# zhiyuns/REHRSeg

Measured on AMD Instinct MI355X. Metric: 3D patches/sec (fwd+bwd, 128^3 fp32), higher is better.
Workload: dtype f32; 1 GPU; FLAVR UNet_3D_3D(1,'unet_18',128,4) fwd+bwd+Adam, 1x1x128^3 patch per GPU, random-init weights; patches_per_gpu=1, global_batch=1, parallelism=dp1 (patch-parallel, flat-bucket RCCL all-reduce), wgrad_stream=True

## Files before the change

include/rehrseg_hip.h:

```cpp
#ifndef REHRSEG_HIP_H
#define REHRSEG_HIP_H

#include <stdint.h>

#ifdef __cplusplus
extern "C" {
#endif

#define REHR_OK 0
#define REHR_EINVAL -1
#define REHR_ENOSUP -2
#define REHR_EHIP -3

#define REHR_ACT_NONE 0
#define REHR_ACT_RELU 1
#define REHR_ACT_LRELU 2

typedef struct {
  int32_t count, off0, offs, k0, ks;
} rehr_axis_taps;

typedef struct {
  const float* x1;
  const float* x2;
// ... 39 lines not shown
#define REHR_GG_ROUTE_FLAT8 1
#define REHR_GG_ROUTE_W32P 2
#define REHR_GG_ROUTE_BIG8 3
#define REHR_GG_ROUTE_SMALL 4
#define REHR_GG_ROUTE_FLAT22 5
#define REHR_GG_ROUTE_REGION22 6
int rehr_gather_gemm_wino_route(const rehr_gather_gemm_desc* d);
#define REHR_GG_DIRECT_NONE 0
#define REHR_GG_DIRECT_GENERIC 1
#define REHR_GG_DIRECT_HALO 2
#define REHR_GG_DIRECT_TCONV_KS 3
int rehr_gather_gemm_direct_route(const rehr_gather_gemm_desc* descs, int32_t count, int32_t bf16, int32_t* routes);
int rehr_gather_gemm_f32(const rehr_gather_gemm_desc* d, void* stream);
int rehr_gather_gemm_multi_f32(const rehr_gather_gemm_desc* descs, int32_t count,
                               void* stream);
int rehr_gather_gemm_bf16(const rehr_gather_gemm_desc* d, void* stream);
int rehr_gather_gemm_multi_bf16(const rehr_gather_gemm_desc* descs, int32_t count, void* stream);
int rehr_pack_weights_bf16(const float* in, void* out, int32_t A, int32_t Apad, int32_t B, int32_t T,
                           int32_t transpose_ab, void* stream);

int rehr_sum_slabs_bias_act_f32(const float* slabs, int32_t S, int64_t slab_stride,
                                const float* bias, float* y, int64_t rows, int32_t C,
                                int32_t act, float slope, void* stream);

int rehr_sum_slabs_stats_f32(const float* slabs, int32_t S, int64_t slab_stride, const float* bias,
                             float* y, int32_t N, int64_t SV, int32_t C, int32_t act, float slope,
                             double* stats, void* stream);

int rehr_sum_slabs_bias_act_bf16(const float* slabs, int32_t S, int64_t slab_stride, const float* bias, void* y,
                                 int64_t rows, int32_t C, int32_t act, float slope, void* stream);
// ... 326 lines not shown
```

rehrseg_amd/csrc/gather_gemm.hip:

```cpp
#include "common.h"
#include "halo_shared.h"
#include "wino_shared.h"

namespace {

constexpr int BK = 32;
constexpr int LDS_LD = 36;
constexpr int NTHREADS = 256;

template <int BM, int BN, int WGM, int WGN, int LDSBUF>
__device__ __forceinline__ void gather_gemm_body(const GGParams& p, const int nblocks, const int logical_in = -1) {
  constexpr int WTM = BM / WGM, WTN = BN / WGN;
  constexpr int FM = WTM / 32, FN = WTN / 32;
  constexpr int AROWS = BM / 32, BROWS = BN / 32;
  static_assert(WGM * WGN == 4, "4 waves");
  const rehr_gather_gemm_desc& d = p.d;

  extern __shared__ __attribute__((aligned(16))) float smem[];
  float* As = smem;
  float* Bs = smem + LDSBUF * BM * LDS_LD;
  int* row_out = (int*)(Bs + LDSBUF * BN * LDS_LD);

  const int tid = threadIdx.x;
  const int lane = tid & 63, wave = tid >> 6;
// ... 290 lines not shown
  if (npad % 64 == 0) return launch_gg<128, 64, 2, 2, 1>(pm, count, st);
  return launch_gg<128, 32, 4, 1, 1>(pm, count, st);
}

}

WinoRoute wino_route(const rehr_gather_gemm_desc& d, WinoPlan& plan) {
  if (!(d.debug_flags & REHR_DBG_GG_NO_FLAT8) && wino_flat8_plan(d, plan)) return WINO_FLAT8;
  if (const WinoRoute r = wino_region_plan(d, plan)) return r;
  if (wino22_flat_plan(d, plan, 1)) return WINO_FLAT22;
  if (wino22_region_plan(d, plan)) return WINO_REGION22;
  plan.bytes = 0;
  return WINO_NONE;
}

static int wino_run(WinoRoute r, const rehr_gather_gemm_desc* ds, int count, const WinoPlan& plan, hipStream_t st) {
  for (int i = 0; i < count; ++i) {
    const int rc = r >= WINO_FLAT22 ? wino22_weights_launch(ds[i], plan, st) : wino_weights_launch(r, ds[i], plan, st);
    if (rc != REHR_OK) return rc;
  }
  if (ds[0].flags & REHR_GG_WS_ONLY) return REHR_OK;
  switch (r) {
    case WINO_FLAT8: return wino_flat8_launch(ds[0], plan, st);
    case WINO_W32P: case WINO_BIG8: case WINO_SMALL: return wino_region_launch(r, ds, count, plan, st);
    default: return wino22_launch(r, ds, count, plan, st);
  }
}

extern "C" int rehr_gather_gemm_multi_f32(const rehr_gather_gemm_desc* descs, int32_t count, void* stream) {
  DirectRoute route[MAX_PHASES];
  const int rrc = direct_route(descs, count, 4, route);
  if (rrc != REHR_OK) return rrc;
  hipStream_t st = (hipStream_t)stream;
  const bool ws_only = (descs[0].flags & REHR_GG_WS_ONLY) != 0;
  for (int i = 1; i < count; ++i)
    if ((descs[i].flags ^ descs[0].flags) & (REHR_GG_WS_ONLY | REHR_GG_WS_READY)) return REHR_EINVAL;
  if (route[0].kind == DIRECT_TCONV_KS && !ws_only) return tconv_ks_launch(descs, count, false, st);
  WinoPlan plan{};
  if (count > 1 && descs[0].wino_ws != nullptr) {
    const int taps = descs[0].td.count;
    if ((taps > 3 || taps == 1) && wino_split_plan(descs, count, plan)) return wino_run(WINO_BIG8, descs, count, plan, st);
    if (taps <= 3 && wino22_flat_multi_plan(descs, count, plan)) return wino_run(WINO_FLAT22, descs, count, plan, st);
  }
  GGMulti pm;
  pm.interleave = 0;
  pm.count = 0;
  pm.no_interleave = (descs[0].debug_flags & REHR_DBG_GG_INTERLEAVE) ? 0 : 1;
  int n = 0;
  for (int i = 0; i < count; ++i) {
    if (descs[i].wino_ws != nullptr && !(count > 1 && descs[i].td.count > 3)) {
      const WinoRoute r = wino_route(descs[i], plan);
      if (r != WINO_NONE && wino_ws_ok(descs[i], plan.bytes)) {
        const int wrc = wino_run(r, &descs[i], 1, plan, st);
        if (wrc != REHR_OK) return wrc;
        continue;
      }
    }
    if (ws_only) continue;
    if (route[i].kind == DIRECT_HALO) {
      const int hrc = halo_f32_launch(route[i].halo, st);
      if (hrc != REHR_OK) return hrc;
    } else if (route[i].kind == DIRECT_GENERIC) {
      pm.ph[n++] = route[i].gg;
    } else {
      return REHR_ENOSUP;
    }
  }
  if (n == 0) return REHR_OK;
  return launch_generic(pm, n, st);
}

extern "C" int64_t rehr_gather_gemm_wino_bytes(const rehr_gather_gemm_desc* dp) {
  WinoPlan plan{};
  if (dp == nullptr || validate(*dp) != REHR_OK || wino_route(*dp, plan) == WINO_NONE) return 0;
  return plan.bytes;
}

extern "C" int rehr_gather_gemm_wino_route(const rehr_gather_gemm_desc* dp) {
  WinoPlan plan{};
  if (dp == nullptr || validate(*dp) != REHR_OK) return REHR_GG_ROUTE_NONE;
  const WinoRoute r = wino_route(*dp, plan);
  return r == WINO_NONE ? REHR_GG_ROUTE_NONE : (int)r | (plan.variant << 8);
}

extern "C" int rehr_gather_gemm_direct_route(const rehr_gather_gemm_desc* descs, int32_t count, int32_t bf16,
                                             int32_t* routes) {
// ... 13 lines not shown
```

rehrseg_amd/csrc/wino22_conv.hip:

```cpp
#include "common.h"
#include "wino_shared.h"
#include <cstdlib>

namespace {

constexpr int LD = WINO_LDX;
constexpr int PW = 17;
constexpr int RP = PW * LD + 12;
constexpr int BUF = PW * RP;
constexpr int PVOX = PW * PW;
constexpr int NT_ = 768;
constexpr int NX = (PVOX * 8 + NT_ - 1) / NT_;
constexpr int MAXPH = WINO_MAXPH;

struct W22Params {
  rehr_gather_gemm_desc d;
  int nb_h, nb_w, kchunks, nphase;
  Phase phase[MAXPH];
  const float* up;
  uint32_t up_bytes;
};

__global__ void w22_weights_kernel(const rehr_gather_gemm_desc d, float* __restrict__ up, int kchunks) {
  AxisPlan ah, aw;
// ... 8 lines not shown
  for (int64_t i = (int64_t)blockIdx.x * blockDim.x + threadIdx.x; i < total; i += (int64_t)gridDim.x * blockDim.x) {
    const int pj = (int)(i / per);
    const int p = pj / d.td.count, jd = pj - p * d.td.count;
    const int p_h = p / aw.nph, p_w = p - p_h * aw.nph;
    const int64_t rem = i - (int64_t)pj * per;
    const int n = (int)(rem / cpad), ci = (int)(rem - (int64_t)n * cpad);
    float g[2][2];
#pragma unroll
    for (int a = 0; a < 2; ++a)
#pragma unroll
      for (int b = 0; b < 2; ++b) {
        const int wt = ((d.td.k0 + d.td.ks * jd) * d.KH + ah.kidx[p_h][a]) * d.KW + aw.kidx[p_w][b];
        g[a][b] = ci < d.Cin ? d.wp[(int64_t)wt * per_src + (int64_t)n * d.Cin + ci] : 0.f;
      }
    float u[9];
    u[0] = g[0][0];              u[1] = g[0][0] + g[0][1];                     u[2] = g[0][1];
    u[3] = g[0][0] + g[1][0];    u[4] = g[0][0] + g[0][1] + g[1][0] + g[1][1]; u[5] = g[0][1] + g[1][1];
    u[6] = g[1][0];              u[7] = g[1][0] + g[1][1];                     u[8] = g[1][1];
    const int nt = n >> 5, col = n & 31, chunk = ci >> 5, kk = (ci >> 3) & 3, half = (ci >> 2) & 1, e = ci & 3;
#pragma unroll
    for (int x = 0; x < 9; ++x) {
      const int64_t o = (((((int64_t)pj * 9 + x) * NT + nt) * kchunks + chunk) * 4 + kk) * 256 + (half * 32 + col) * 4 + e;
      up[o] = u[x];
    }
  }
}

__global__ __launch_bounds__(NT_) void wino22_conv_kernel(const W22Params p) {
  const rehr_gather_gemm_desc& d = p.d;
  extern __shared__ __attribute__((aligned(16))) float smem[];
  float* Xs = smem;

  const int tid = threadIdx.x, lane = tid & 63;
// ... 629 lines not shown
```

rehrseg_amd/csrc/wino_conv.hip:

```cpp
#include "common.h"
#include "wino_shared.h"
#include <cstdlib>

namespace {

constexpr int TH = 4, TW = 8;
constexpr int PH = 2 * TH + 2, PW = 2 * TW + 2;
constexpr int PVOX = PH * PW;
constexpr int LDX = 36;
constexpr int NX = (PVOX * 8 + 255) / 256;

struct WinoParams {
  rehr_gather_gemm_desc d;
  int nb_h, nb_w;
  int band_major;
  int kchunks;
  int dh0, dw0;
  const float* up;
  uint32_t up_bytes;
  int nsplit;
  rehr_axis_taps s_td[8];
  const float* s_up[8];
  uint32_t s_up_bytes[8];
  float* s_y[8];
};

__global__ void wino_weights_kernel(const rehr_gather_gemm_desc d, float* __restrict__ up) {
  const float G[4][3] = {{1.f, 0.f, 0.f}, {.5f, .5f, .5f}, {.5f, -.5f, .5f}, {0.f, 0.f, 1.f}};
  const int64_t per = (int64_t)d.Npad * d.Cin;
  const int64_t total = (int64_t)d.td.count * per;
  for (int64_t i = (int64_t)blockIdx.x * blockDim.x + threadIdx.x; i < total; i += (int64_t)gridDim.x * blockDim.x) {
    const int jd = (int)(i / per);
    const int64_t nc = i - (int64_t)jd * per;
    float g[3][3];
#pragma unroll
    for (int jh = 0; jh < 3; ++jh)
#pragma unroll
      for (int jw = 0; jw < 3; ++jw) {
        const int a = d.bh + d.th.off0 + d.th.offs * jh + 1;
        const int b = d.bw + d.tw.off0 + d.tw.offs * jw + 1;
        const int wt = ((d.td.k0 + d.td.ks * jd) * d.KH + (d.th.k0 + d.th.ks * jh)) * d.KW + (d.tw.k0 + d.tw.ks * jw);
        const float v = d.wp[(int64_t)wt * per + nc];
#pragma unroll
        for (int aa = 0; aa < 3; ++aa)
#pragma unroll
          for (int bb = 0; bb < 3; ++bb)
            if (aa == a && bb == b) g[aa][bb] = v;
      }
    float t[4][3];
#pragma unroll
    for (int r = 0; r < 4; ++r)
#pragma unroll
      for (int b = 0; b < 3; ++b) t[r][b] = G[r][0] * g[0][b] + G[r][1] * g[1][b] + G[r][2] * g[2][b];
#pragma unroll
    for (int r = 0; r < 4; ++r)
#pragma unroll
      for (int c = 0; c < 4; ++c)
        up[((int64_t)jd * 16 + r * 4 + c) * per + nc] = t[r][0] * G[c][0] + t[r][1] * G[c][1] + t[r][2] * G[c][2];
  }
}

__global__ __launch_bounds__(256, 2) void wino_conv_kernel(const WinoParams p) {
  const rehr_gather_gemm_desc& d = p.d;
  extern __shared__ __attribute__((aligned(16))) float smem[];
  float* Xs = smem;

  const int tid = threadIdx.x, lane = tid & 63;
  const int r = __builtin_amdgcn_readfirstlane(tid >> 6);
  const int half = lane >> 5, col = lane & 31;
  const int n_img = blockIdx.z;
  const int n0 = blockIdx.y * 32;
  int b = xcd_remap(blockIdx.x, gridDim.x);
  const int bw_ = b % p.nb_w; b /= p.nb_w;
// ... 169 lines not shown
    if (r == 0 && half == 0 && colok) {
      const float a1 = red[col] + red[64 + col] + red[128 + col] + red[192 + col];
      const float a2 = red[32 + col] + red[96 + col] + red[160 + col] + red[224 + col];
      double* st = d.stats + ((int64_t)n_img * d.Cout + col_n) * 2;
      atomicAdd(st, (double)a1);
      if (d.stats_mode == 2) atomicAdd(st + 1, (double)a2);
    }
  }
}

constexpr int PW2 = 18, PVOX2 = 18 * 18;
constexpr int RP2 = PW2 * LDX + 8;
constexpr int BUF2 = PW2 * RP2;

__global__ void wino_weights_frag_kernel(const rehr_gather_gemm_desc d, float* __restrict__ up, int kchunks) {
  const float G[4][3] = {{1.f, 0.f, 0.f}, {.5f, .5f, .5f}, {.5f, -.5f, .5f}, {0.f, 0.f, 1.f}};
  const int cpad = kchunks * 32;
  const int64_t per = (int64_t)d.Npad * cpad;
  const int64_t per_src = (int64_t)d.Npad * d.Cin;
  const int64_t total = (int64_t)d.td.count * per;
  const int NT = d.Npad / 32;
  for (int64_t i = (int64_t)blockIdx.x * blockDim.x + threadIdx.x; i < total; i += (int64_t)gridDim.x * blockDim.x) {
    const int jd = (int)(i / per);
    const int64_t rem = i - (int64_t)jd * per;
    const int n = (int)(rem / cpad), ci = (int)(rem - (int64_t)n * cpad);
    float g[3][3];
#pragma unroll
    for (int jh = 0; jh < 3; ++jh)
#pragma unroll
      for (int jw = 0; jw < 3; ++jw) {
        const int a = d.bh + d.th.off0 + d.th.offs * jh + 1;
        const int b = d.bw + d.tw.off0 + d.tw.offs * jw + 1;
        const int wt = ((d.td.k0 + d.td.ks * jd) * d.KH + (d.th.k0 + d.th.ks * jh)) * d.KW + (d.tw.k0 + d.tw.ks * jw);
        const float v = ci < d.Cin ? d.wp[(int64_t)wt * per_src + (int64_t)n * d.Cin + ci] : 0.f;
#pragma unroll
        for (int aa = 0; aa < 3; ++aa)
#pragma unroll
          for (int bb = 0; bb < 3; ++bb)
            if (aa == a && bb == b) g[aa][bb] = v;
      }
    float t[4][3];
#pragma unroll
    for (int r = 0; r < 4; ++r)
#pragma unroll
      for (int b = 0; b < 3; ++b) t[r][b] = G[r][0] * g[0][b] + G[r][1] * g[1][b] + G[r][2] * g[2][b];
    const int nt = n >> 5, col = n & 31, chunk = ci >> 5, kk = (ci >> 3) & 3, half = (ci >> 2) & 1, e = ci & 3;
#pragma unroll
    for (int r = 0; r < 4; ++r)
#pragma unroll
      for (int c = 0; c < 4; ++c) {
        const int64_t o = (((((int64_t)jd * 16 + r * 4 + c) * NT + nt) * kchunks + chunk) * 4 + kk) * 256 +
                          (half * 32 + col) * 4 + e;
        up[o] = t[r][0] * G[c][0] + t[r][1] * G[c][1] + t[r][2] * G[c][2];
      }
  }
}

constexpr int NX8 = (PVOX2 * 8 + 511) / 512;

__global__ __launch_bounds__(512) void wino_conv_big8_kernel(const WinoParams p) {
  const rehr_gather_gemm_desc& d = p.d;
  extern __shared__ __attribute__((aligned(16))) float smem[];
  float* Xs = smem;
  constexpr int BUF = BUF2;

  const int tid = threadIdx.x, lane = tid & 63;
  const int wv = __builtin_amdgcn_readfirstlane(tid >> 6);
  const int r = wv & 3, fm = wv >> 2;
  const int half = lane >> 5, col = lane & 31;
// ... 694 lines not shown
```

rehrseg_amd/csrc/wino_shared.h:

```cpp
#pragma once
#include "common.h"
#include "gg_shared.h"
#include "wino22_shared.h"

enum WinoRoute {
  WINO_NONE = REHR_GG_ROUTE_NONE,
  WINO_FLAT8 = REHR_GG_ROUTE_FLAT8,
  WINO_W32P = REHR_GG_ROUTE_W32P,
  WINO_BIG8 = REHR_GG_ROUTE_BIG8,
  WINO_SMALL = REHR_GG_ROUTE_SMALL,
  WINO_FLAT22 = REHR_GG_ROUTE_FLAT22,
  WINO_REGION22 = REHR_GG_ROUTE_REGION22,
};

constexpr int WINO_LDX = 36;
constexpr int WINO_MAXPH = 4;

struct Phase {
  int sh, sw;
  int ph, pw;
  int dh0, dw0;
};

struct FlatGeom {
// ... 112 lines not shown
    return a.count == b.count && a.off0 == b.off0 && a.offs == b.offs && a.k0 == b.k0 && a.ks == b.ks;
  };
  if ((groups & SAME_HW_TAPS) && (d.bh != d0.bh || d.bw != d0.bw || d.KH != d0.KH || d.KW != d0.KW ||
                                  !same_axis(d.th, d0.th) || !same_axis(d.tw, d0.tw)))
    return false;
  if ((groups & SAME_DEPTH_TAPS) && (d.td.count != d0.td.count || d.td.off0 != d0.td.off0 || d.td.offs != d0.td.offs))
    return false;
  if ((groups & SAME_DEST) &&
      (d.y != d0.y || d.Dy != d0.Dy || d.Hy != d0.Hy || d.Wy != d0.Wy || d.osd != d0.osd || d.osh != d0.osh ||
       d.osw != d0.osw || d.obd != d0.obd || d.bias != d0.bias || d.act != d0.act || d.slope != d0.slope ||
       d.stats != d0.stats || d.stats_mode != d0.stats_mode))
    return false;
  return true;
}

template <auto KERN, typename... Args>
static int wino_transform_launch(const rehr_gather_gemm_desc& d, int64_t total, int cap, hipStream_t stream, Args... args) {
  if (d.flags & REHR_GG_WS_READY) return REHR_OK;
  int64_t blocks = (total + 255) / 256;
  if (blocks > cap) blocks = cap;
  hipLaunchKernelGGL(KERN, dim3((unsigned)blocks), dim3(256), 0, stream, d, d.wino_ws, args...);
  REHR_LAUNCH_CHECK();
  return REHR_OK;
}

WinoRoute wino_region_plan(const rehr_gather_gemm_desc& d, WinoPlan& plan);
bool wino_split_plan(const rehr_gather_gemm_desc* ds, int count, WinoPlan& plan);
int wino_weights_launch(WinoRoute r, const rehr_gather_gemm_desc& d, const WinoPlan& plan, hipStream_t stream);
int wino_region_launch(WinoRoute r, const rehr_gather_gemm_desc* ds, int count, const WinoPlan& plan, hipStream_t stream);
bool wino_flat8_plan(const rehr_gather_gemm_desc& d, WinoPlan& plan);
int wino_flat8_launch(const rehr_gather_gemm_desc& d, const WinoPlan& plan, hipStream_t stream);
bool wino22_flat_plan(const rehr_gather_gemm_desc& d, WinoPlan& plan, int parts);
bool wino22_region_plan(const rehr_gather_gemm_desc& d, WinoPlan& plan);
bool wino22_flat_multi_plan(const rehr_gather_gemm_desc* ds, int count, WinoPlan& plan);
int wino22_weights_launch(const rehr_gather_gemm_desc& d, const WinoPlan& plan, hipStream_t stream);
int wino22_launch(WinoRoute r, const rehr_gather_gemm_desc* ds, int count, const WinoPlan& plan, hipStream_t stream);
```

rehrseg_amd/hip_backend.py:

```python
from __future__ import annotations

import ctypes as C
import os
import functools
import weakref

import torch
from torch.optim.optimizer import register_optimizer_step_post_hook as _register_step_hook

from . import lib as L

name = "hip"


def _stream():
    return C.c_void_p(torch.cuda.current_stream().cuda_stream)


_prof = None


def profile_start():
    global _prof
    _prof = []
# ... 203 lines not shown
        return (p if part is None else p.narrow(*part)).contiguous()

    if not _keeps_forms(w):
        out = torch.empty((T, Apad, B), dtype=dtype, device=w.device)
        _pack_launch(src(w), out, A, Apad, B, T, transpose)
        return out
    key = ("pack", id(w), tuple(w.shape), part, A, Apad, B, T, bool(transpose), dtype)
    f = _forms.get(key)
    if f is None or f.param() is not w:
        out = torch.empty((T, Apad, B), dtype=dtype, device=w.device)
        f = _forms[key] = _Form(key, w, lambda p: _pack_launch(src(p), out, A, Apad, B, T, transpose))
        f.out = out
        _form_of_panel[id(out)] = f
    _form_ready(f, w)
    return f.out


USE_WINOGRAD = True
USE_WINOGRAD_WGRAD = True
USE_HALO_BF16 = True
WGRAD_TAP_COLOCATE = True
USE_WGRAD_TAP_SKIP = True
W32P_BLOCKS = 0
PHASE_INTERLEAVE = False
WINO_BAND_MAJOR = True
USE_TCONV_KS = True
USE_WINO_FLAT8 = True
WINO_FLAT8_TILES = 0
wino_wgrad_launches = 0
wino_launches = 0
# ... 79 lines not shown
            cp[i].flags |= L.GG_WS_ONLY

        def make(_p, cp=cp, n=n):
            L.check(L.load().rehr_gather_gemm_multi_f32(cp, n, _stream()), "rehr_gather_gemm_multi_f32 (weight forms)")

        f = _forms[key] = _Form(key, p, make, dep=pf)
        f.out = outs
    _form_ready(f, p)
    for i in range(n):
        if needs[i]:
            descs[i].wino_ws, descs[i].wino_ws_bytes = _ptr(f.out[i]), needs[i]
        descs[i].flags |= L.GG_WS_READY
    return f.out


def _gg_tag(arr, n=1, bf16=False):
    d = arr[0]
    name = _ROUTE_NAMES.get(wino_route(d)[0]) if d.wino_ws else None
    if name is None:
        try:
            kinds = [_DIRECT_NAMES[bf16].get(r, "none") for r in direct_route(arr, n, bf16)]
            name = "+".join(sorted(set(kinds), key=kinds.index))
        except L.RehrsegHipError:
            name = "invalid"
    return (f"N{d.N} {d.Cin}->{d.Cout} lattice {d.Ld}x{d.Lh}x{d.Lw} stride {d.sd}{d.sh}{d.sw} "
            f"taps {d.td.count}x{d.th.count}x{d.tw.count}" + (" +x2" if d.x2 else "") + f" [{name}]")


_ROUTE_NAMES = {L.GG_ROUTE_FLAT8: "flat8", L.GG_ROUTE_W32P: "w32p", L.GG_ROUTE_BIG8: "big8", L.GG_ROUTE_SMALL: "small",
                L.GG_ROUTE_FLAT22: "flat22", L.GG_ROUTE_REGION22: "region22"}
# ... 14 lines not shown
    r = int(L.load().rehr_gather_gemm_wino_route(C.byref(d)))
    return r & 255, (r >> 8) & 255


def _gg_family(d):
    if _prof is None:
        return None
    if not d.wino_ws:
        return "gather_gemm"
    route = wino_route(d)[0]
    if route == L.GG_ROUTE_NONE:
        return "gather_gemm"
    return "wino22_conv" if route in (L.GG_ROUTE_FLAT22, L.GG_ROUTE_REGION22) else "wino_conv"


def gather_gemm(*args):
    d = L.GatherGemmDesc()
    flops = _gg_desc(d, *args)
    if args[0].dtype == torch.bfloat16:
        with _timed("gather_gemm_bf16", flops, lambda: _gg_tag((L.GatherGemmDesc * 1)(d), bf16=True)):
            L.check(L.load().rehr_gather_gemm_bf16(C.byref(d), _stream()), "rehr_gather_gemm_bf16")
        return
    arr = (L.GatherGemmDesc * 1)(d)
    keep = _attach_ws(arr, 1, [_gg_desc.need], [_gg_desc.sig], args[11])
    with _timed(_gg_family(arr[0]), flops, lambda: _gg_tag(arr)):
        L.check(L.load().rehr_gather_gemm_multi_f32(arr, 1, _stream()), "rehr_gather_gemm_f32")
    del keep


def gather_gemm_multi(calls):
    if len(calls) == 1:
        return gather_gemm(*calls[0])
    arr = (L.GatherGemmDesc * len(calls))()
    flops, needs, sigs = 0.0, [], []
    for i, a in enumerate(calls):
        flops += _gg_desc(arr[i], *a)
        needs.append(_gg_desc.need)
        sigs.append(_gg_desc.sig)
    if calls[0][0].dtype == torch.bfloat16:
        with _timed("gather_gemm_bf16", flops, lambda: f"{len(calls)} parts of " + _gg_tag(arr, len(calls), bf16=True)):
            L.check(L.load().rehr_gather_gemm_multi_bf16(arr, len(calls), _stream()), "rehr_gather_gemm_multi_bf16")
        return
    keep = _attach_ws(arr, len(calls), needs, sigs, calls[0][11])
    with _timed(_gg_family(arr[0]) if all(arr[i].wino_ws for i in range(len(calls))) else "gather_gemm", flops,
                lambda: f"{len(calls)} parts of " + _gg_tag(arr, len(calls))):
        L.check(L.load().rehr_gather_gemm_multi_f32(arr, len(calls), _stream()), "rehr_gather_gemm_multi_f32")
    del keep


def sum_slabs_bias_act(slabs, S, bias, act, slope, stats=None, out_dtype=None):
    _chk_dev(slabs, bias, f64=(stats,))
    if slabs.dtype != torch.float32:
        raise L.RehrsegHipError("split-K slabs are float32")
    SN, Cc, D, H, W = slabs.shape
    N = SN // S
    bf = out_dtype == torch.bfloat16
    y = new_act(N, Cc, D, H, W, like=slabs, dtype=torch.bfloat16 if bf else torch.float32)
    rows = N * D * H * W
# ... 935 lines not shown
```

rehrseg_amd/lib.py:

```python
from __future__ import annotations

import ctypes as C
import os
import re
from typing import Optional

_HERE = os.path.dirname(os.path.abspath(__file__))
LIB_PATH = os.environ.get("REHRSEG_HIP_LIB") or os.path.join(_HERE, "librehrseg_hip.so")
HEADER_PATH = os.path.join(os.path.dirname(_HERE), "include", "rehrseg_hip.h")

ACT_NONE, ACT_RELU, ACT_LRELU = 0, 1, 2
ABI_VERSION = 6
GG_Y_F32 = 1
GG_WS_READY = 2
GG_WS_ONLY = 4
DBG_WGRAD_DIRECT = 1
DBG_WGRAD_NO_TAP_SKIP = 2
DBG_WGRAD_NO_TAP_COLOCATE = 4
DBG_GG_NO_HALO = 1
DBG_GG_NO_FLAT8 = 2
DBG_GG_FLAT8_HALF = 4
DBG_GG_FLAT8_FULL = 8
DBG_GG_W32P_TWO_PER_CU = 16
DBG_GG_W32P_ONE_PER_CU = 32
# ... 83 lines not shown
                ("d", _i32), ("h", _i32), ("w", _i32), ("ld", _i32), ("ldd", _i32), ("weight", _f32)]


class PyramidLevel(C.Structure):
    _fields_ = [("dst", _vp), ("d", _i32), ("h", _i32), ("w", _i32), ("iz", _vp), ("iy", _vp), ("ix", _vp)]


_P_GG, _P_WG, _P_DC =C.POINTER(GatherGemmDesc), C.POINTER(WgradDesc), C.POINTER(DirectConvDesc)

PROTOTYPES = {
    "rehr_gather_gemm_wino_bytes": (_i64, [_P_GG]),
    "rehr_gather_gemm_wino_route": (C.c_int, [_P_GG]),
    "rehr_gather_gemm_direct_route": (C.c_int, [_P_GG, _i32, _i32, C.POINTER(_i32)]),
    "rehr_gather_gemm_f32": (C.c_int, [_P_GG, _vp]),
    "rehr_gather_gemm_multi_f32": (C.c_int, [_P_GG, _i32, _vp]),
    "rehr_gather_gemm_bf16": (C.c_int, [_P_GG, _vp]),
    "rehr_gather_gemm_multi_bf16": (C.c_int, [_P_GG, _i32, _vp]),
    "rehr_pack_weights_bf16": (C.c_int, [_vp, _vp, _i32, _i32, _i32, _i32, _i32, _vp]),
    "rehr_sum_slabs_bias_act_f32": (C.c_int, [_vp, _i32, _i64, _vp, _vp, _i64, _i32, _i32, _f32, _vp]),
    "rehr_sum_slabs_stats_f32": (C.c_int, [_vp, _i32, _i64, _vp, _vp, _i32, _i64, _i32, _i32, _f32, _vp, _vp]),
    "rehr_sum_slabs_bias_act_bf16": (C.c_int, [_vp, _i32, _i64, _vp, _vp, _i64, _i32, _i32, _f32, _vp]),
    "rehr_sum_slabs_stats_bf16": (C.c_int, [_vp, _i32, _i64, _vp, _vp, _i32, _i64, _i32, _i32, _f32, _vp, _vp]),
    "rehr_wgrad_workspace_bytes": (_i64, [_P_WG]),
    "rehr_wgrad_uses_winograd": (C.c_int, [_P_WG]),
    "rehr_wgrad_f32": (C.c_int, [_P_WG, _vp]),
    "rehr_wgrad_bf16_workspace_bytes": (_i64, [_P_WG]),
    "rehr_wgrad_bf16": (C.c_int, [_P_WG, _vp]),
    "rehr_pack_weights_f32": (C.c_int, [_vp, _vp, _i32, _i32, _i32, _i32, _i32, _vp]),
    "rehr_conv_small_cin_fwd_f32": (C.c_int, [_P_DC, _vp]),
    "rehr_im2col_f32": (C.c_int, [_P_DC, _vp, _i32, _vp]),
# ... 144 lines not shown
```

rehrseg_amd/ops.py:

```python
from __future__ import annotations

import functools
import itertools
import weakref
from dataclasses import dataclass
from typing import Optional, Tuple

import torch

from . import hip_backend

ACT_NONE, ACT_RELU, ACT_LRELU = 0, 1, 2

_backend = hip_backend


def get_backend():
    return _backend


def set_backend(b):
    global _backend
    old = _backend
    _backend = b
# ... 109 lines not shown
        return tuple((i - 1) * s - 2 * p + k for i, k, s, p in zip(in_dims, K, cfg.stride, cfg.pad))
    return tuple(conv_out_dim(i, k, s, p) for i, k, s, p in zip(in_dims, K, cfg.stride, cfg.pad))


def _pack(w, dest_dim, dtype=torch.float32, part=None):
    be = get_backend()
    T = w.shape[2] * w.shape[3] * w.shape[4]
    kw = {"dtype": torch.bfloat16} if dtype == torch.bfloat16 else {}
    shape = list(w.shape)
    if part is not None:
        if hasattr(be, "invalidate_weight_forms"):
            kw["part"] = part
        else:
            w = w.narrow(*part).contiguous()
        shape[part[0]] = part[2]
    if dest_dim == 0:
        A, B = shape[0], shape[1]
        return be.pack_weights(w, A, pad_rows(A), B, T, False, **kw), pad_rows(A)
    A, B = shape[1], shape[0]
    return be.pack_weights(w, A, pad_rows(A), B, T, True, **kw), pad_rows(A)


def _phased_gather(src1, src2, c1, Csrc, wp, Npad, dst, Cdst, K, stride, pad, bias, act, slope, stats, stats_mode):
    be = get_backend()
    src_dims, dst_dims = _spatial(src1), _spatial(dst)
    calls = []
    for ph in itertools.product(*(range(s) for s in stride)):
        taps = [phase_taps(K[a], stride[a], pad[a], ph[a]) for a in range(3)]
        lattice = tuple((dst_dims[a] - ph[a] + stride[a] - 1) // stride[a] for a in range(3))
        if min(lattice) <= 0:
            continue
        if any(t is None for t in taps):
            continue
        thin = tuple(src_dims[a] == 1 and taps[a][0] > 1 for a in range(3))
        calls.append((src1, src2, c1, src_dims, Csrc, lattice, (1, 1, 1), (0, 0, 0), taps, K[1], K[2], wp, Npad,
# ... 506 lines not shown
```

Before: 16.79 patches/s.

## Build Winograd weight forms in one pass directly from raw conv weights

Adds a new kernel that reads the raw 5D conv weight tensor, stages taps in LDS, and writes the Winograd-transformed (F33 fragment, F33 plain or F22 fragment) weight forms directly. This skips the separate pack_weights panel and the later per-phase transform launches. The Python side defers panel packing through a lazy wrapper and falls back to the old pack path when the one-pass route is unsupported. The aim is to cut a launch and a full weight-panel round trip through memory on every step, at the cost of more routing code and an added LDS-staged kernel.

```diff
diff --git a/include/rehrseg_hip.h b/include/rehrseg_hip.h
--- a/include/rehrseg_hip.h
+++ b/include/rehrseg_hip.h
@@ -77,6 +77,9 @@
 int rehr_gather_gemm_f32(const rehr_gather_gemm_desc* d, void* stream);
 int rehr_gather_gemm_multi_f32(const rehr_gather_gemm_desc* descs, int32_t count,
                                void* stream);
+int rehr_gather_gemm_wino_forms_f32(const rehr_gather_gemm_desc* descs, int32_t count, const float* w, int32_t D0,
+                                    int32_t D1, int32_t T, int32_t dest_dim, int32_t dest_lo, int32_t src_lo,
+                                    void* stream);
 int rehr_gather_gemm_bf16(const rehr_gather_gemm_desc* d, void* stream);
 int rehr_gather_gemm_multi_bf16(const rehr_gather_gemm_desc* descs, int32_t count, void* stream);
 int rehr_pack_weights_bf16(const float* in, void* out, int32_t A, int32_t Apad, int32_t B, int32_t T,
diff --git a/rehrseg_amd/csrc/gather_gemm.hip b/rehrseg_amd/csrc/gather_gemm.hip
--- a/rehrseg_amd/csrc/gather_gemm.hip
+++ b/rehrseg_amd/csrc/gather_gemm.hip
@@ -328,6 +328,20 @@
   return WINO_NONE;
 }
 
+static WinoRoute wino_joint_route(const rehr_gather_gemm_desc* descs, int count, WinoPlan& plan) {
+  if (count > 1 && descs[0].wino_ws != nullptr) {
+    const int taps = descs[0].td.count;
+    if ((taps > 3 || taps == 1) && wino_split_plan(descs, count, plan)) return WINO_BIG8;
+    if (taps <= 3 && wino22_flat_multi_plan(descs, count, plan)) return WINO_FLAT22;
+  }
+  return WINO_NONE;
+}
+static WinoRoute wino_part_route(const rehr_gather_gemm_desc& d, int count, WinoPlan& plan) {
+  if (d.wino_ws == nullptr || (count > 1 && d.td.count > 3)) return WINO_NONE;
+  const WinoRoute r = wino_route(d, plan);
+  return r != WINO_NONE && wino_ws_ok(d, plan.bytes) ? r : WINO_NONE;
+}
+
 static int wino_run(WinoRoute r, const rehr_gather_gemm_desc* ds, int count, const WinoPlan& plan, hipStream_t st) {
   for (int i = 0; i < count; ++i) {
     const int rc = r >= WINO_FLAT22 ? wino22_weights_launch(ds[i], plan, st) : wino_weights_launch(r, ds[i], plan, st);
@@ -351,24 +365,17 @@
     if ((descs[i].flags ^ descs[0].flags) & (REHR_GG_WS_ONLY | REHR_GG_WS_READY)) return REHR_EINVAL;
   if (route[0].kind == DIRECT_TCONV_KS && !ws_only) return tconv_ks_launch(descs, count, false, st);
   WinoPlan plan{};
-  if (count > 1 && descs[0].wino_ws != nullptr) {
-    const int taps = descs[0].td.count;
-    if ((taps > 3 || taps == 1) && wino_split_plan(descs, count, plan)) return wino_run(WINO_BIG8, descs, count, plan, st);
-    if (taps <= 3 && wino22_flat_multi_plan(descs, count, plan)) return wino_run(WINO_FLAT22, descs, count, plan, st);
-  }
+  if (const WinoRoute joint = wino_joint_route(descs, count, plan)) return wino_run(joint, descs, count, plan, st);
   GGMulti pm;
   pm.interleave = 0;
   pm.count = 0;
   pm.no_interleave = (descs[0].debug_flags & REHR_DBG_GG_INTERLEAVE) ? 0 : 1;
   int n = 0;
   for (int i = 0; i < count; ++i) {
-    if (descs[i].wino_ws != nullptr && !(count > 1 && descs[i].td.count > 3)) {
-      const WinoRoute r = wino_route(descs[i], plan);
-      if (r != WINO_NONE && wino_ws_ok(descs[i], plan.bytes)) {
-        const int wrc = wino_run(r, &descs[i], 1, plan, st);
-        if (wrc != REHR_OK) return wrc;
-        continue;
-      }
+    if (const WinoRoute r = wino_part_route(descs[i], count, plan)) {
+      const int wrc = wino_run(r, &descs[i], 1, plan, st);
+      if (wrc != REHR_OK) return wrc;
+      continue;
     }
     if (ws_only) continue;
     if (route[i].kind == DIRECT_HALO) {
@@ -384,6 +391,43 @@
   return launch_generic(pm, n, st);
 }
 
+extern "C" int rehr_gather_gemm_wino_forms_f32(const rehr_gather_gemm_desc* descs, int32_t count, const float* w,
+                                               int32_t D0, int32_t D1, int32_t T, int32_t dest_dim, int32_t dest_lo,
+                                               int32_t src_lo, void* stream) {
+  if (w == nullptr || ((uintptr_t)w & 3) || D0 < 1 || D1 < 1 || T < 1 || (dest_dim != 0 && dest_dim != 1) || dest_lo < 0 ||
+      src_lo < 0)
+    return REHR_EINVAL;
+  DirectRoute route[MAX_PHASES];
+  const int rrc = direct_route(descs, count, 4, route);
+  if (rrc != REHR_OK) return rrc;
+  const int Ddest = dest_dim == 0 ? D0 : D1, Dsrc = dest_dim == 0 ? D1 : D0;
+  for (int i = 0; i < count; ++i) {
+    const rehr_gather_gemm_desc& d = descs[i];
+    if (d.Cout > Ddest - dest_lo || d.Cin > Dsrc - src_lo) return REHR_EINVAL;
+    if (d.KH < 1 || d.KW < 1 || T % (d.KH * d.KW)) return REHR_EINVAL;
+    const rehr_axis_taps* ax[3] = {&d.td, &d.th, &d.tw};
+    const int ext[3] = {T / (d.KH * d.KW), d.KH, d.KW};
+    for (int a = 0; a < 3; ++a) {
+      const int64_t first = ax[a]->k0, last = (int64_t)ax[a]->k0 + (int64_t)ax[a]->ks * (ax[a]->count - 1);
+      if (first < 0 || first >= ext[a] || last < 0 || last >= ext[a]) return REHR_EINVAL;
+    }
+  }
+  if (route[0].kind == DIRECT_TCONV_KS) return REHR_ENOSUP;
+  WinoRoute r[MAX_PHASES];
+  WinoPlan plan{};
+  const WinoRoute joint = wino_joint_route(descs, count, plan);
+  for (int i = 0; i < count; ++i) {
+    r[i] = joint ? joint : wino_part_route(descs[i], count, plan);
+    if (r[i] == WINO_NONE) return REHR_ENOSUP;
+  }
+  WinoWeightSrc src;
+  const int64_t s0 = (int64_t)D1 * T, s1 = T;
+  src.sn = dest_dim == 0 ? s0 : s1;
+  src.sc = dest_dim == 0 ? s1 : s0;
+  src.w = w + dest_lo * src.sn + src_lo * src.sc;
+  return wino_forms_launch(r, descs, count, src, (hipStream_t)stream);
+}
+
 extern "C" int64_t rehr_gather_gemm_wino_bytes(const rehr_gather_gemm_desc* dp) {
   WinoPlan plan{};
   if (dp == nullptr || validate(*dp) != REHR_OK || wino_route(*dp, plan) == WINO_NONE) return 0;
diff --git a/rehrseg_amd/csrc/wino22_conv.hip b/rehrseg_amd/csrc/wino22_conv.hip
--- a/rehrseg_amd/csrc/wino22_conv.hip
+++ b/rehrseg_amd/csrc/wino22_conv.hip
@@ -46,9 +46,7 @@
         g[a][b] = ci < d.Cin ? d.wp[(int64_t)wt * per_src + (int64_t)n * d.Cin + ci] : 0.f;
       }
     float u[9];
-    u[0] = g[0][0];              u[1] = g[0][0] + g[0][1];                     u[2] = g[0][1];
-    u[3] = g[0][0] + g[1][0];    u[4] = g[0][0] + g[0][1] + g[1][0] + g[1][1]; u[5] = g[0][1] + g[1][1];
-    u[6] = g[1][0];              u[7] = g[1][0] + g[1][1];                     u[8] = g[1][1];
+    wino_u22(g, u);
     const int nt = n >> 5, col = n & 31, chunk = ci >> 5, kk = (ci >> 3) & 3, half = (ci >> 2) & 1, e = ci & 3;
 #pragma unroll
     for (int x = 0; x < 9; ++x) {
diff --git a/rehrseg_amd/csrc/wino_conv.hip b/rehrseg_amd/csrc/wino_conv.hip
--- a/rehrseg_amd/csrc/wino_conv.hip
+++ b/rehrseg_amd/csrc/wino_conv.hip
@@ -26,7 +26,6 @@
 };
 
 __global__ void wino_weights_kernel(const rehr_gather_gemm_desc d, float* __restrict__ up) {
-  const float G[4][3] = {{1.f, 0.f, 0.f}, {.5f, .5f, .5f}, {.5f, -.5f, .5f}, {0.f, 0.f, 1.f}};
   const int64_t per = (int64_t)d.Npad * d.Cin;
   const int64_t total = (int64_t)d.td.count * per;
   for (int64_t i = (int64_t)blockIdx.x * blockDim.x + threadIdx.x; i < total; i += (int64_t)gridDim.x * blockDim.x) {
@@ -47,16 +46,10 @@
           for (int bb = 0; bb < 3; ++bb)
             if (aa == a && bb == b) g[aa][bb] = v;
       }
-    float t[4][3];
-#pragma unroll
-    for (int r = 0; r < 4; ++r)
-#pragma unroll
-      for (int b = 0; b < 3; ++b) t[r][b] = G[r][0] * g[0][b] + G[r][1] * g[1][b] + G[r][2] * g[2][b];
-#pragma unroll
-    for (int r = 0; r < 4; ++r)
-#pragma unroll
-      for (int c = 0; c < 4; ++c)
-        up[((int64_t)jd * 16 + r * 4 + c) * per + nc] = t[r][0] * G[c][0] + t[r][1] * G[c][1] + t[r][2] * G[c][2];
+    float u[16];
+    wino_u33(g, u);
+#pragma unroll
+    for (int xi = 0; xi < 16; ++xi) up[((int64_t)jd * 16 + xi) * per + nc] = u[xi];
   }
 }
 
@@ -256,7 +249,6 @@
 constexpr int BUF2 = PW2 * RP2;
 
 __global__ void wino_weights_frag_kernel(const rehr_gather_gemm_desc d, float* __restrict__ up, int kchunks) {
-  const float G[4][3] = {{1.f, 0.f, 0.f}, {.5f, .5f, .5f}, {.5f, -.5f, .5f}, {0.f, 0.f, 1.f}};
   const int cpad = kchunks * 32;
   const int64_t per = (int64_t)d.Npad * cpad;
   const int64_t per_src = (int64_t)d.Npad * d.Cin;
@@ -281,20 +273,14 @@
           for (int bb = 0; bb < 3; ++bb)
             if (aa == a && bb == b) g[aa][bb] = v;
       }
-    float t[4][3];
-#pragma unroll
-    for (int r = 0; r < 4; ++r)
-#pragma unroll
-      for (int b = 0; b < 3; ++b) t[r][b] = G[r][0] * g[0][b] + G[r][1] * g[1][b] + G[r][2] * g[2][b];
+    float u[16];
+    wino_u33(g, u);
     const int nt = n >> 5, col = n & 31, chunk = ci >> 5, kk = (ci >> 3) & 3, half = (ci >> 2) & 1, e = ci & 3;
 #pragma unroll
-    for (int r = 0; r < 4; ++r)
-#pragma unroll
-      for (int c = 0; c < 4; ++c) {
-        const int64_t o = (((((int64_t)jd * 16 + r * 4 + c) * NT + nt) * kchunks + chunk) * 4 + kk) * 256 +
-                          (half * 32 + col) * 4 + e;
-        up[o] = t[r][0] * G[c][0] + t[r][1] * G[c][1] + t[r][2] * G[c][2];
-      }
+    for (int xi = 0; xi < 16; ++xi) {
+      const int64_t o = (((((int64_t)jd * 16 + xi) * NT + nt) * kchunks + chunk) * 4 + kk) * 256 + (half * 32 + col) * 4 + e;
+      up[o] = u[xi];
+    }
   }
 }
 
diff --git a/rehrseg_amd/csrc/wino_forms.hip b/rehrseg_amd/csrc/wino_forms.hip
--- /dev/null
+++ b/rehrseg_amd/csrc/wino_forms.hip
@@ -0,0 +1,187 @@
+#include "common.h"
+#include "wino_shared.h"
+
+namespace {
+
+enum FormKind { FORM_F33_FRAG = 0, FORM_F33_PLAIN = 1, FORM_F22_FRAG = 2 };
+
+struct FormPart {
+  float* up;
+  int npj;
+  int nd;
+  int doff0, dstep;
+  int hw[16];
+};
+struct FormParams {
+  const float* w;
+  int64_t sn, sc;
+  int inner_ci;
+  int A, Cin, Npad, kchunks;
+  FormPart part[MAX_PHASES];
+};
+
+constexpr int FORM_ROW = 33;
+
+template <int KIND>
+__global__ __launch_bounds__(256) void wino_forms_kernel(const FormParams p) {
+  constexpr int NTAP = KIND == FORM_F22_FRAG ? 4 : 9, TP = NTAP | 1, NX = KIND == FORM_F22_FRAG ? 9 : 16;
+  __shared__ float sg[32 * FORM_ROW * TP];
+  const FormPart& q = p.part[blockIdx.z];
+  const int pj = blockIdx.y;
+  if (pj >= q.npj) return;
+  const int ph = pj / q.nd, jd = pj - ph * q.nd;
+  const int nt = blockIdx.x / p.kchunks, chunk = blockIdx.x - nt * p.kchunks;
+  const int tid = threadIdx.x;
+  const int64_t toff = (int64_t)q.doff0 + (int64_t)q.dstep * jd;
+  const int hw0 = KIND == FORM_F22_FRAG ? ph * 4 : 0;
+
+  __shared__ int shw[16];
+  if (tid < 16) shw[tid] = q.hw[tid];
+  __syncthreads();
+  float v[4 * NTAP];
+#pragma unroll
+  for (int i = 0; i < 4 * NTAP; ++i) {
+    const int s = i * 256 + tid;
+    const int it = s / NTAP, j = s - it * NTAP;
+    const int in = it & 31, out = it >> 5;
+    const int n = nt * 32 + (p.inner_ci ? out : in), ci = chunk * 32 + (p.inner_ci ? in : out);
+    v[i] = 0.f;
+    if (n < p.A && ci < p.Cin) v[i] = p.w[(int64_t)n * p.sn + (int64_t)ci * p.sc + toff + shw[hw0 + j]];
+  }
+#pragma unroll
+  for (int i = 0; i < 4 * NTAP; ++i) {
+    const int s = i * 256 + tid;
+    const int it = s / NTAP, j = s - it * NTAP;
+    const int in = it & 31, out = it >> 5;
+    const int n_l = p.inner_ci ? out : in, ci_l = p.inner_ci ? in : out;
+    sg[(ci_l * FORM_ROW + n_l) * TP + j] = v[i];
+  }
+  __syncthreads();
+
+#pragma unroll
+  for (int k = 0; k < 4; ++k) {
+    int n_l, ci_l;
+    if (KIND == FORM_F33_PLAIN) {
+      n_l = k * 8 + (tid >> 5);
+      ci_l = tid & 31;
+    } else {
+      const int lane = tid >> 2, e = tid & 3;
+      n_l = lane & 31;
+      ci_l = k * 8 + (lane >> 5) * 4 + e;
+    }
+    const float* gp = sg + (ci_l * FORM_ROW + n_l) * TP;
+    float u[NX];
+    if constexpr (KIND == FORM_F22_FRAG) {
+      float g[2][2];
+#pragma unroll
+      for (int a = 0; a < 2; ++a)
+#pragma unroll
+        for (int b = 0; b < 2; ++b) g[a][b] = gp[a * 2 + b];
+      wino_u22(g, u);
+    } else {
+      float g[3][3];
+#pragma unroll
+      for (int a = 0; a < 3; ++a)
+#pragma unroll
+        for (int b = 0; b < 3; ++b) g[a][b] = gp[a * 3 + b];
+      wino_u33(g, u);
+    }
+    if (KIND == FORM_F33_PLAIN) {
+      const int n = nt * 32 + n_l, ci = chunk * 32 + ci_l;
+      const int64_t per = (int64_t)p.Npad * p.Cin;
+      if (ci < p.Cin) {
+        float* o = q.up + (int64_t)jd * 16 * per + (int64_t)n * p.Cin + ci;
+#pragma unroll
+        for (int x = 0; x < NX; ++x) o[x * per] = u[x];
+      }
+    } else {
+      const int64_t xs = (int64_t)(p.Npad / 32) * p.kchunks * 1024;
+      float* o = q.up + (int64_t)pj * NX * xs + ((int64_t)nt * p.kchunks + chunk) * 1024 + k * 256 + tid;
+#pragma unroll
+      for (int x = 0; x < NX; ++x) o[x * xs] = u[x];
+    }
+  }
+}
+
+FormKind form_kind(WinoRoute r) {
+  return r >= WINO_FLAT22 ? FORM_F22_FRAG : r == WINO_SMALL ? FORM_F33_PLAIN : FORM_F33_FRAG;
+}
+
+bool fill_part(FormKind kind, const rehr_gather_gemm_desc& d, FormPart& q) {
+  const int khw = d.KH * d.KW;
+  q.up = d.wino_ws;
+  q.nd = d.td.count;
+  q.doff0 = d.td.k0 * khw;
+  q.dstep = d.td.ks * khw;
+  for (int i = 0; i < 16; ++i) q.hw[i] = 0;
+  if (kind == FORM_F22_FRAG) {
+    AxisPlan ah, aw;
+    if (!plan_axis(d.th, d.sh, d.bh, ah) || !plan_axis(d.tw, d.sw, d.bw, aw) || ah.nph * aw.nph > WINO_MAXPH) return false;
+    q.npj = ah.nph * aw.nph * d.td.count;
+    for (int p_h = 0; p_h < ah.nph; ++p_h)
+      for (int p_w = 0; p_w < aw.nph; ++p_w)
+        for (int a = 0; a < 2; ++a)
+          for (int b = 0; b < 2; ++b)
+            q.hw[(p_h * aw.nph + p_w) * 4 + a * 2 + b] = ah.kidx[p_h][a] * d.KW + aw.kidx[p_w][b];
+    return true;
+  }
+  if (d.th.count != 3 || d.tw.count != 3) return false;
+  q.npj = d.td.count;
+  bool seen[9] = {false};
+  for (int jh = 0; jh < 3; ++jh)
+    for (int jw = 0; jw < 3; ++jw) {
+      const int a = d.bh + d.th.off0 + d.th.offs * jh + 1;
+      const int b = d.bw + d.tw.off0 + d.tw.offs * jw + 1;
+      if (a < 0 || a > 2 || b < 0 || b > 2) return false;
+      q.hw[a * 3 + b] = (d.th.k0 + d.th.ks * jh) * d.KW + (d.tw.k0 + d.tw.ks * jw);
+      seen[a * 3 + b] = true;
+    }
+  for (int i = 0; i < 9; ++i)
+    if (!seen[i]) return false;
+  return true;
+}
+
+template <int KIND>
+void launch_forms(const FormParams& p, int parts, int max_pj, hipStream_t stream) {
+  dim3 grid((unsigned)((p.Npad / 32) * p.kchunks), (unsigned)max_pj, (unsigned)parts);
+  hipLaunchKernelGGL(wino_forms_kernel<KIND>, grid, dim3(256), 0, stream, p);
+}
+
+}
+
+int wino_forms_launch(const WinoRoute* r, const rehr_gather_gemm_desc* ds, int count, const WinoWeightSrc& src,
+                      hipStream_t stream) {
+  if (count < 1 || count > MAX_PHASES) return REHR_EINVAL;
+  bool done[MAX_PHASES] = {false};
+  FormPart parts[MAX_PHASES];
+  for (int i = 0; i < count; ++i) {
+    if (r[i] == WINO_NONE) return REHR_ENOSUP;
+    if (!fill_part(form_kind(r[i]), ds[i], parts[i]) || parts[i].npj < 1 || parts[i].npj > 65535) return REHR_EINVAL;
+  }
+  for (int i = 0; i < count; ++i) {
+    if (done[i]) continue;
+    const FormKind kind = form_kind(r[i]);
+    FormParams p;
+    p.w = src.w;
+    p.sn = src.sn;
+    p.sc = src.sc;
+    p.inner_ci = src.sc < src.sn ? 1 : 0;
+    p.A = ds[i].Cout;
+    p.Cin = ds[i].Cin;
+    p.Npad = ds[i].Npad;
+    p.kchunks = (ds[i].Cin + 31) / 32;
+    int n = 0, max_pj = 0;
+    for (int j = i; j < count; ++j) {
+      if (done[j] || form_kind(r[j]) != kind || ds[j].Cout != p.A || ds[j].Cin != p.Cin || ds[j].Npad != p.Npad) continue;
+      done[j] = true;
+      p.part[n++] = parts[j];
+      if (parts[j].npj > max_pj) max_pj = parts[j].npj;
+    }
+    for (int j = n; j < MAX_PHASES; ++j) p.part[j] = p.part[0];
+    if (kind == FORM_F22_FRAG) launch_forms<FORM_F22_FRAG>(p, n, max_pj, stream);
+    else if (kind == FORM_F33_PLAIN) launch_forms<FORM_F33_PLAIN>(p, n, max_pj, stream);
+    else launch_forms<FORM_F33_FRAG>(p, n, max_pj, stream);
+    REHR_LAUNCH_CHECK();
+  }
+  return REHR_OK;
+}
diff --git a/rehrseg_amd/csrc/wino_shared.h b/rehrseg_amd/csrc/wino_shared.h
--- a/rehrseg_amd/csrc/wino_shared.h
+++ b/rehrseg_amd/csrc/wino_shared.h
@@ -150,6 +150,24 @@
   return true;
 }
 
+__device__ __forceinline__ void wino_u33(const float (&g)[3][3], float (&u)[16]) {
+  const float G[4][3] = {{1.f, 0.f, 0.f}, {.5f, .5f, .5f}, {.5f, -.5f, .5f}, {0.f, 0.f, 1.f}};
+  float t[4][3];
+#pragma unroll
+  for (int r = 0; r < 4; ++r)
+#pragma unroll
+    for (int b = 0; b < 3; ++b) t[r][b] = G[r][0] * g[0][b] + G[r][1] * g[1][b] + G[r][2] * g[2][b];
+#pragma unroll
+  for (int r = 0; r < 4; ++r)
+#pragma unroll
+    for (int c = 0; c < 4; ++c) u[r * 4 + c] = t[r][0] * G[c][0] + t[r][1] * G[c][1] + t[r][2] * G[c][2];
+}
+__device__ __forceinline__ void wino_u22(const float (&g)[2][2], float (&u)[9]) {
+  u[0] = g[0][0];              u[1] = g[0][0] + g[0][1];                     u[2] = g[0][1];
+  u[3] = g[0][0] + g[1][0];    u[4] = g[0][0] + g[0][1] + g[1][0] + g[1][1]; u[5] = g[0][1] + g[1][1];
+  u[6] = g[1][0];              u[7] = g[1][0] + g[1][1];                     u[8] = g[1][1];
+}
+
 template <auto KERN, typename... Args>
 static int wino_transform_launch(const rehr_gather_gemm_desc& d, int64_t total, int cap, hipStream_t stream, Args... args) {
   if (d.flags & REHR_GG_WS_READY) return REHR_OK;
@@ -171,3 +189,10 @@
 bool wino22_flat_multi_plan(const rehr_gather_gemm_desc* ds, int count, WinoPlan& plan);
 int wino22_weights_launch(const rehr_gather_gemm_desc& d, const WinoPlan& plan, hipStream_t stream);
 int wino22_launch(WinoRoute r, const rehr_gather_gemm_desc* ds, int count, const WinoPlan& plan, hipStream_t stream);
+
+struct WinoWeightSrc {
+  const float* w;
+  int64_t sn, sc;
+};
+int wino_forms_launch(const WinoRoute* r, const rehr_gather_gemm_desc* ds, int count, const WinoWeightSrc& src,
+                      hipStream_t stream);
diff --git a/rehrseg_amd/hip_backend.py b/rehrseg_amd/hip_backend.py
--- a/rehrseg_amd/hip_backend.py
+++ b/rehrseg_amd/hip_backend.py
@@ -241,6 +241,55 @@
         _form_of_panel[id(out)] = f
     _form_ready(f, w)
     return f.out
+
+
+USE_ONEPASS_FORMS = True
+onepass_form_calls = 0
+
+
+class _LazyPanel:
+    __slots__ = ("w", "A", "Apad", "B", "T", "transpose", "part", "_out")
+
+    def __init__(self, w, A, Apad, B, T, transpose, part):
+        self.w, self.A, self.Apad, self.B, self.T, self.transpose, self.part = w, A, Apad, B, T, bool(transpose), part
+        self._out = None
+
+    def panel(self):
+        if self._out is None:
+            self._out = pack_weights(self.w, self.A, self.Apad, self.B, self.T, self.transpose, part=self.part)
+        return self._out
+
+
+def lazy_weights(w, A, Apad, B, T, transpose, part=None):
+    _chk_dev(w)
+    if (not USE_ONEPASS_FORMS or not USE_WINOGRAD or _keeps_forms(w) or w.dtype != torch.float32 or w.dim() != 5 or
+            not w.is_contiguous()):
+        return pack_weights(w, A, Apad, B, T, transpose, part=part)
+    return _LazyPanel(w, A, Apad, B, T, transpose, part)
+
+
+def _onepass_forms(arr, n, needs, lazy):
+    global onepass_form_calls
+    if not all(needs) or any(arr[i].Cout != lazy.A or arr[i].Cin != lazy.B for i in range(n)):
+        return None
+    w = lazy.w
+    keep = _attach_ws(arr, n, needs, None, w)
+    dest_dim = 1 if lazy.transpose else 0
+    dest_lo = src_lo = 0
+    if lazy.part is not None:
+        if lazy.part[0] == dest_dim:
+            dest_lo = lazy.part[1]
+        else:
+            src_lo = lazy.part[1]
+    rc = L.load().rehr_gather_gemm_wino_forms_f32(arr, n, _ptr(w), w.shape[0], w.shape[1], lazy.T, dest_dim, dest_lo,
+                                                  src_lo, _stream())
+    if rc == -2:
+        return keep, False
+    L.check(rc, "rehr_gather_gemm_wino_forms_f32")
+    for i in range(n):
+        arr[i].flags |= L.GG_WS_READY
+    onepass_form_calls += 1
+    return keep, True
 
 
 USE_WINOGRAD = True
@@ -350,6 +399,16 @@
     return f.out
 
 
+def _lazy_ws(arr, n, needs, lazy):
+    got = _onepass_forms(arr, n, needs, lazy)
+    if got is not None and got[1]:
+        return got[0]
+    panel = lazy.panel()
+    _set_panel(arr, n, panel)
+    keep = got[0] if got is not None else _attach_ws(arr, n, needs, None, panel)
+    return (keep, panel)
+
+
 def _gg_tag(arr, n=1, bf16=False):
     d = arr[0]
     name = _ROUTE_NAMES.get(wino_route(d)[0]) if d.wino_ws else None
@@ -394,7 +453,19 @@
     return "wino22_conv" if route in (L.GG_ROUTE_FLAT22, L.GG_ROUTE_REGION22) else "wino_conv"
 
 
+def _with_wp(args, wp):
+    return args[:11] + (wp,) + args[12:]
+
+
+def _set_panel(arr, n, panel):
+    for i in range(n):
+        arr[i].wp = _ptr(panel)
+
+
 def gather_gemm(*args):
+    lazy = args[11] if isinstance(args[11], _LazyPanel) else None
+    if lazy is not None:
+        args = _with_wp(args, lazy.w)
     d = L.GatherGemmDesc()
     flops = _gg_desc(d, *args)
     if args[0].dtype == torch.bfloat16:
@@ -402,7 +473,8 @@
             L.check(L.load().rehr_gather_gemm_bf16(C.byref(d), _stream()), "rehr_gather_gemm_bf16")
         return
     arr = (L.GatherGemmDesc * 1)(d)
-    keep = _attach_ws(arr, 1, [_gg_desc.need], [_gg_desc.sig], args[11])
+    keep = _lazy_ws(arr, 1, [_gg_desc.need], lazy) if lazy is not None else \
+        _attach_ws(arr, 1, [_gg_desc.need], [_gg_desc.sig], args[11])
     with _timed(_gg_family(arr[0]), flops, lambda: _gg_tag(arr)):
         L.check(L.load().rehr_gather_gemm_multi_f32(arr, 1, _stream()), "rehr_gather_gemm_f32")
     del keep
@@ -411,6 +483,9 @@
 def gather_gemm_multi(calls):
     if len(calls) == 1:
         return gather_gemm(*calls[0])
+    lazy = calls[0][11] if isinstance(calls[0][11], _LazyPanel) else None
+    if lazy is not None:
+        calls = [_with_wp(a, lazy.w) for a in calls]
     arr = (L.GatherGemmDesc * len(calls))()
     flops, needs, sigs = 0.0, [], []
     for i, a in enumerate(calls):
@@ -421,7 +496,8 @@
         with _timed("gather_gemm_bf16", flops, lambda: f"{len(calls)} parts of " + _gg_tag(arr, len(calls), bf16=True)):
             L.check(L.load().rehr_gather_gemm_multi_bf16(arr, len(calls), _stream()), "rehr_gather_gemm_multi_bf16")
         return
-    keep = _attach_ws(arr, len(calls), needs, sigs, calls[0][11])
+    keep = _lazy_ws(arr, len(calls), needs, lazy) if lazy is not None else \
+        _attach_ws(arr, len(calls), needs, sigs, calls[0][11])
     with _timed(_gg_family(arr[0]) if all(arr[i].wino_ws for i in range(len(calls))) else "gather_gemm", flops,
                 lambda: f"{len(calls)} parts of " + _gg_tag(arr, len(calls))):
         L.check(L.load().rehr_gather_gemm_multi_f32(arr, len(calls), _stream()), "rehr_gather_gemm_multi_f32")
diff --git a/rehrseg_amd/lib.py b/rehrseg_amd/lib.py
--- a/rehrseg_amd/lib.py
+++ b/rehrseg_amd/lib.py
@@ -121,6 +121,7 @@
     "rehr_gather_gemm_direct_route": (C.c_int, [_P_GG, _i32, _i32, C.POINTER(_i32)]),
     "rehr_gather_gemm_f32": (C.c_int, [_P_GG, _vp]),
     "rehr_gather_gemm_multi_f32": (C.c_int, [_P_GG, _i32, _vp]),
+    "rehr_gather_gemm_wino_forms_f32": (C.c_int, [_P_GG, _i32, _vp, _i32, _i32, _i32, _i32, _i32, _i32, _vp]),
     "rehr_gather_gemm_bf16": (C.c_int, [_P_GG, _vp]),
     "rehr_gather_gemm_multi_bf16": (C.c_int, [_P_GG, _i32, _vp]),
     "rehr_pack_weights_bf16": (C.c_int, [_vp, _vp, _i32, _i32, _i32, _i32, _i32, _vp]),
diff --git a/rehrseg_amd/ops.py b/rehrseg_amd/ops.py
--- a/rehrseg_amd/ops.py
+++ b/rehrseg_amd/ops.py
@@ -147,11 +147,12 @@
         else:
             w = w.narrow(*part).contiguous()
         shape[part[0]] = part[2]
+    pack = getattr(be, "lazy_weights", be.pack_weights) if dtype != torch.bfloat16 else be.pack_weights
     if dest_dim == 0:
         A, B = shape[0], shape[1]
-        return be.pack_weights(w, A, pad_rows(A), B, T, False, **kw), pad_rows(A)
+        return pack(w, A, pad_rows(A), B, T, False, **kw), pad_rows(A)
     A, B = shape[1], shape[0]
-    return be.pack_weights(w, A, pad_rows(A), B, T, True, **kw), pad_rows(A)
+    return pack(w, A, pad_rows(A), B, T, True, **kw), pad_rows(A)
 
 
 def _phased_gather(src1, src2, c1, Csrc, wp, Npad, dst, Cdst, K, stride, pad, bias, act, slope, stats, stats_mode):
```

Measured after the change: 17.05 patches/s, median of 6. 1.02x the previous value.
